# menyifang/MIMO

Measured on NVIDIA H100. Metric: frames/sec @ 512x512x24f, 20 DDIM steps, higher is better.
Workload: dtype fp16

## Files before the change

### include/mimo_b200.h

```cpp
#ifndef MIMO_B200_H_
#define MIMO_B200_H_

#include <stdint.h>

#ifdef __cplusplus
extern "C" {
#endif

#define MIMO_OK 0
#define MIMO_ERR_ARG (-1)
#define MIMO_ERR_CUDA (-2)
#define MIMO_ERR_DEVICE (-3)

#define MIMO_F16 0
#define MIMO_BF16 1

#define MIMO_ACT_NONE 0
#define MIMO_ACT_SILU 1
#define MIMO_ACT_GEGLU 2

const char* mimo_version(void);
const char* mimo_last_error(void);
int mimo_device_check(int dev);
int mimo_abi_sizeof(int which);
// ... 83 lines not shown
  void* out;
  int64_t ld_out;
  int32_t n, lq, heads, d;
  float scale;
  int32_t dtype;
} mimo_attn_params;
int mimo_attn_spatial(const mimo_attn_params* p, void* stream);

typedef struct {
  const void* q;
  int64_t ld_q;
  const void* k;
  const void* v;
  int64_t ld_kv;
  void* out;
  int64_t ld_out;
  int64_t chunk_stride_rows;
  int32_t batch, q_frames, kv_frames, frames_per_chunk;
  int32_t hw, heads, d;
  float scale;
  int32_t dtype;
} mimo_attn_temporal_params;
int mimo_attn_temporal(const mimo_attn_temporal_params* p, void* stream);

#define MIMO_MAX_PEERS 8
typedef struct {
  const void* peer_src[MIMO_MAX_PEERS];
  void* peer_ready[MIMO_MAX_PEERS];
  void* ctl;
  void* dst;
  const void* residual;
  int32_t mode, G, r;
  int32_t b, fl, hw, C;
  int32_t dtype;
  int32_t max_blocks;
  int32_t timeout_ms;
} mimo_exchange_params;
int mimo_exchange(const mimo_exchange_params* p, void* stream);
int mimo_peer_alloc(int64_t bytes, void** ptr, void* handle64);
int mimo_peer_open(const void* handle64, void** ptr);
int mimo_peer_close(void* ptr);
int mimo_peer_free(void* ptr);

int mimo_ncfhw_to_nhwc(const void* src, void* dst, int32_t b, int32_t c, int32_t f, int32_t h, int32_t w,
                       int32_t cpad, int32_t src_is_f32, int32_t dtype, void* stream);
int mimo_nhwc_to_ncfhw(const void* src, void* dst, int32_t b, int32_t c, int32_t f, int32_t h, int32_t w,
// ... 48 lines not shown
```

### mimo_b200/csrc/attn_temporal.cu

```cuda
#include <cuda_runtime.h>

#include "../../include/mimo_b200.h"
#include "host_util.h"
#include "ptx.cuh"

namespace mimo {

struct TemporalArgs {
  const void* q;
  const void* k;
  const void* v;
  void* out;
  long long ld_q, ld_kv, ld_out, chunk_stride_rows;
  int Fq, F, fpc, hw, heads, d;
  int dpad;
  int hg;
  int pitch;
  float scale_log2;
};

__device__ __forceinline__ void ldsm_x4(uint32_t (&r)[4], const void* p) {
  asm volatile("ldmatrix.sync.aligned.m8n8.x4.shared.b16 {%0, %1, %2, %3}, [%4];"
               : "=r"(r[0]), "=r"(r[1]), "=r"(r[2]), "=r"(r[3])
               : "r"(smem_u32(p)));
}
__device__ __forceinline__ void ldsm_x4_trans(uint32_t (&r)[4], const void* p) {
  asm volatile("ldmatrix.sync.aligned.m8n8.x4.trans.shared.b16 {%0, %1, %2, %3}, [%4];"
               : "=r"(r[0]), "=r"(r[1]), "=r"(r[2]), "=r"(r[3])
               : "r"(smem_u32(p)));
}
__device__ __forceinline__ void cp_async16(void* smem_dst, const void* gmem_src) {
  asm volatile("cp.async.cg.shared.global [%0], [%1], 16;" ::"r"(smem_u32(smem_dst)), "l"(gmem_src) : "memory");
}
template <bool kBf16>
__device__ __forceinline__ void mma16816(float (&c)[4], const uint32_t (&a)[4], uint32_t b0, uint32_t b1) {
  if constexpr (kBf16) {
    asm volatile("mma.sync.aligned.m16n8k16.row.col.f32.bf16.bf16.f32 {%0, %1, %2, %3}, {%4, %5, %6, %7}, {%8, %9}, "
                 "{%0, %1, %2, %3};"
                 : "+f"(c[0]), "+f"(c[1]), "+f"(c[2]), "+f"(c[3])
                 : "r"(a[0]), "r"(a[1]), "r"(a[2]), "r"(a[3]), "r"(b0), "r"(b1));
  } else {
    asm volatile("mma.sync.aligned.m16n8k16.row.col.f32.f16.f16.f32 {%0, %1, %2, %3}, {%4, %5, %6, %7}, {%8, %9}, "
                 "{%0, %1, %2, %3};"
                 : "+f"(c[0]), "+f"(c[1]), "+f"(c[2]), "+f"(c[3])
                 : "r"(a[0]), "r"(a[1]), "r"(a[2]), "r"(a[3]), "r"(b0), "r"(b1));
  }
}

template <bool kBf16, int D, int HG>
__global__ void __launch_bounds__(1024) attn_temporal_kernel(TemporalArgs a_in) {
  pdl_launch_dependents();
  pdl_wait();
  TemporalArgs a = a_in;
  if constexpr (D > 0) {
    a.d = D;
    a.dpad = (D + 15) / 16 * 16;
    a.hg = HG;
    a.pitch = HG * ((D + 15) / 16 * 16) + 8;
  }
  using C = Cvt<kBf16>;
  using T = typename C::T;
  extern __shared__ uint4 smem_qkv[];
  T* sq = reinterpret_cast<T*>(smem_qkv);
  T* sk = sq + 32 * a.pitch;
  T* sv = sk + 32 * a.pitch;
  const int groups = a.heads / a.hg;
  const int hg0 = (blockIdx.x % groups) * a.hg;
  const int bp = blockIdx.x / groups;
  const int b = bp / a.hw;
  const int p = bp % a.hw;
  const int d = a.d, dpad = a.dpad, pitch = a.pitch;
// ... 27 lines not shown
      }
    }
  }
  {
    const int warp = threadIdx.x >> 5, lane = threadIdx.x & 31, nwarps = blockDim.x >> 5;
    if (dpad > d) {
      const int padv = (dpad - d) / 8;
      for (int f = warp; f < 32; f += nwarps)
        for (int hh = lane; hh < a.hg; hh += 32)
          for (int pc = 0; pc < padv; ++pc) {
            *reinterpret_cast<uint4*>(sq + f * pitch + hh * dpad + d + pc * 8) = make_uint4(0, 0, 0, 0);
            *reinterpret_cast<uint4*>(sk + f * pitch + hh * dpad + d + pc * 8) = make_uint4(0, 0, 0, 0);
          }
    }
    for (int f = a.F + warp; f < 32; f += nwarps)
      for (int pc = lane; pc < pitch / 8; pc += 32) *reinterpret_cast<uint4*>(sv + f * pitch + pc * 8) = make_uint4(0, 0, 0, 0);
  }
  asm volatile("cp.async.wait_all;" ::: "memory");
  __syncthreads();

  const int hh = threadIdx.x >> 5;
  const int lane = threadIdx.x & 31;
  if (hh >= a.hg) return;
  const int g = lane >> 2, t = lane & 3;
  const int MT = (a.Fq + 15) >> 4;
  const int NT = (a.F + 7) >> 3;
  const bool ragged = (a.F & 7) != 0;
  const T* qh = sq + hh * dpad;
  const T* kh = sk + hh * dpad;
  const T* vh = sv + hh * dpad;

  float s[2][4][4];
#pragma unroll
  for (int mt = 0; mt < 2; ++mt)
#pragma unroll
    for (int nt = 0; nt < 4; ++nt)
#pragma unroll
      for (int e = 0; e < 4; ++e) s[mt][nt][e] = 0.f;
  for (int ks = 0; ks < dpad / 16; ++ks) {
    uint32_t af[2][4];
#pragma unroll
    for (int mt = 0; mt < 2; ++mt)
      if (mt < MT) ldsm_x4(af[mt], qh + (mt * 16 + (lane & 7) + ((lane >> 3) & 1) * 8) * pitch + ks * 16 + (lane >> 4) * 8);
#pragma unroll
    for (int np = 0; np < 2; ++np) {
      if (np * 2 < NT) {
        uint32_t bf[4];
        ldsm_x4(bf, kh + (np * 16 + (lane & 7) + (lane >> 4) * 8) * pitch + ks * 16 + ((lane >> 3) & 1) * 8);
#pragma unroll
        for (int mt = 0; mt < 2; ++mt) {
          if (mt < MT) {
            mma16816<kBf16>(s[mt][np * 2], af[mt], bf[0], bf[1]);
            if (np * 2 + 1 < NT) mma16816<kBf16>(s[mt][np * 2 + 1], af[mt], bf[2], bf[3]);
          }
        }
      }
    }
  }

  float inv_sum[2][2];
  uint32_t pf[2][2][4];
#pragma unroll
  for (int mt = 0; mt < 2; ++mt) {
#pragma unroll
    for (int half = 0; half < 2; ++half) {
      float m = -INFINITY;
#pragma unroll
      for (int nt = 0; nt < 4; ++nt) {
        if (nt < NT) {
#pragma unroll
          for (int e = 0; e < 2; ++e) {
            float& v = s[mt][nt][half * 2 + e];
            v *= a.scale_log2;
            if (ragged && nt == NT - 1 && nt * 8 + 2 * t + e >= a.F) v = -INFINITY;
            m = fmaxf(m, v);
          }
        }
      }
      m = fmaxf(m, __shfl_xor_sync(0xffffffffu, m, 1));
      m = fmaxf(m, __shfl_xor_sync(0xffffffffu, m, 2));
      float sum = 0.f;
#pragma unroll
      for (int nt = 0; nt < 4; ++nt) {
        if (nt < NT) {
#pragma unroll
          for (int e = 0; e < 2; ++e) {
            float& v = s[mt][nt][half * 2 + e];
            asm("ex2.approx.ftz.f32 %0, %1;" : "=f"(v) : "f"(v - m));
            sum += v;
          }
        }
      }
      sum += __shfl_xor_sync(0xffffffffu, sum, 1);
      sum += __shfl_xor_sync(0xffffffffu, sum, 2);
      inv_sum[mt][half] = 1.0f / sum;
    }
#pragma unroll
    for (int kk = 0; kk < 2; ++kk) {
      pf[mt][kk][0] = C::pack(s[mt][2 * kk][0], s[mt][2 * kk][1]);
      pf[mt][kk][1] = C::pack(s[mt][2 * kk][2], s[mt][2 * kk][3]);
      pf[mt][kk][2] = C::pack(s[mt][2 * kk + 1][0], s[mt][2 * kk + 1][1]);
      pf[mt][kk][3] = C::pack(s[mt][2 * kk + 1][2], s[mt][2 * kk + 1][3]);
    }
  }

  __syncwarp();
  T* oh = sq + hh * dpad;
  const int KK = (a.F + 15) >> 4;
  for (int nd = 0; nd < dv; ++nd) {
    uint32_t bv[4];
    ldsm_x4_trans(bv, vh + lane * pitch + nd * 8);
#pragma unroll
    for (int mt = 0; mt < 2; ++mt) {
      if (mt < MT) {
        float o[4] = {0.f, 0.f, 0.f, 0.f};
        mma16816<kBf16>(o, pf[mt][0], bv[0], bv[1]);
        if (KK > 1) mma16816<kBf16>(o, pf[mt][1], bv[2], bv[3]);
        *reinterpret_cast<uint32_t*>(oh + (mt * 16 + g) * pitch + nd * 8 + 2 * t) =
            C::pack(o[0] * inv_sum[mt][0], o[1] * inv_sum[mt][0]);
        *reinterpret_cast<uint32_t*>(oh + (mt * 16 + g + 8) * pitch + nd * 8 + 2 * t) =
            C::pack(o[2] * inv_sum[mt][1], o[3] * inv_sum[mt][1]);
      }
    }
  }
  __syncwarp();
  {
    const int lf = lane / dv, lpc = lane - lf * dv, fstep = 32 / dv;
    if (lf < fstep) {
      for (int f = lf; f < a.Fq; f += fstep) {
        const long long row = (static_cast<long long>(b) * a.Fq + f) * a.hw + p;
        *reinterpret_cast<uint4*>(static_cast<T*>(a.out) + row * a.ld_out + (hg0 + hh) * d + lpc * 8) =
            *reinterpret_cast<const uint4*>(oh + f * pitch + lpc * 8);
      }
    }
  }
}

}

using namespace mimo;

extern "C" int mimo_attn_temporal(const mimo_attn_temporal_params* p, void* stream) {
  if (!p || !p->q || !p->k || !p->v || !p->out) return set_error(MIMO_ERR_ARG, "mimo_attn_temporal: null pointer");
  const int fpc = p->frames_per_chunk > 0 ? p->frames_per_chunk : p->kv_frames;
  if (p->batch <= 0 || p->q_frames <= 0 || p->kv_frames <= 0 || p->kv_frames > 32 || p->q_frames > 32 || p->hw <= 0 ||
      p->heads <= 0 || p->heads > 32 || p->d <= 0 || (p->d % 8) || p->d > 256 || (p->ld_q % 8) || (p->ld_kv % 8) || (p->ld_out % 8) ||
      (p->kv_frames % fpc))
    return set_error(MIMO_ERR_ARG, "mimo_attn_temporal: need frames <= 32, heads <= 32, d % 8 == 0, kv_frames % chunk == 0");
// ... 55 lines not shown
```

### mimo_b200/csrc/capi.cu

```cuda
#include <cudaTypedefs.h>
#include <stdio.h>
#include <string.h>

#include "../../include/mimo_b200.h"
#include "host_util.h"

namespace mimo {

static thread_local char g_err[512] = "";

int set_error(int code, const char* msg) {
  snprintf(g_err, sizeof(g_err), "%s", msg);
  return code;
}
int set_cuda_error(const char* what, cudaError_t e) {
  snprintf(g_err, sizeof(g_err), "%s: %s (%s)", what, cudaGetErrorName(e), cudaGetErrorString(e));
  return MIMO_ERR_CUDA;
}

static int g_dev_state = 0;
static int g_num_sms = 132;

int ensure_device() {
  if (g_dev_state == 1) return MIMO_OK;
// ... 59 lines not shown
             (unsigned long long)(rank > 1 ? gdim[1] : 0), (unsigned long long)(rank > 2 ? gdim[2] : 0),
             (unsigned long long)(rank > 3 ? gdim[3] : 0), bx[0], rank > 1 ? bx[1] : 0, rank > 2 ? bx[2] : 0,
             rank > 3 ? bx[3] : 0, (unsigned long long)(rank > 1 ? gstr[0] : 0));
    return MIMO_ERR_CUDA;
  }
  return MIMO_OK;
}

}

extern "C" const char* mimo_version(void) { return "mimo_b200 0.2.0 (sm_90a)"; }
extern "C" const char* mimo_last_error(void) { return mimo::g_err; }

extern "C" int mimo_abi_sizeof(int which) {
  switch (which) {
    case 0: return static_cast<int>(sizeof(mimo_epilogue));
    case 1: return static_cast<int>(sizeof(mimo_gemm_params));
    case 2: return static_cast<int>(sizeof(mimo_conv3x3_params));
    case 3: return static_cast<int>(sizeof(mimo_groupnorm_params));
    case 4: return static_cast<int>(sizeof(mimo_attn_params));
    case 5: return static_cast<int>(sizeof(mimo_attn_temporal_params));
    case 6: return static_cast<int>(sizeof(mimo_exchange_params));
    case 7: return static_cast<int>(sizeof(mimo_cfg_multistep_params));
  }
  return -1;
}

extern "C" int mimo_device_check(int dev) {
  int count = 0;
  cudaError_t e = cudaGetDeviceCount(&count);
  if (e != cudaSuccess || count == 0) {
    mimo::set_error(MIMO_ERR_DEVICE, "no CUDA device visible; mimo_b200 has no CPU fallback");
    return MIMO_ERR_DEVICE;
  }
  if (dev < 0 || dev >= count) return mimo::set_error(MIMO_ERR_ARG, "mimo_device_check: bad device index");
  int major = 0, minor = 0;
  cudaDeviceGetAttribute(&major, cudaDevAttrComputeCapabilityMajor, dev);
  cudaDeviceGetAttribute(&minor, cudaDevAttrComputeCapabilityMinor, dev);
  if (major != 9 || minor != 0) return mimo::set_error(MIMO_ERR_DEVICE, "device is not sm_90 (H100)");
  return MIMO_OK;
}

extern "C" int mimo_peer_alloc(int64_t bytes, void** ptr, void* handle64) {
  if (!ptr || !handle64 || bytes <= 0) return mimo::set_error(MIMO_ERR_ARG, "mimo_peer_alloc: bad arguments");
  if (int rc = mimo::ensure_device()) return rc;
  void* p = nullptr;
// ... 40 lines not shown
```

### mimo_b200/engine.py

```python
from __future__ import annotations

import math
from dataclasses import dataclass
from typing import Dict, List, Optional, Sequence, Tuple

import torch

from . import lib as L
from . import ops

SD = Dict[str, torch.Tensor]


@dataclass
class UNetSpec:
    block_out_channels: Tuple[int, ...] = (320, 640, 1280, 1280)
    layers_per_block: int = 2
    heads: int = 8
    cross_attention_dim: int = 768
    norm_num_groups: int = 32
    norm_eps: float = 1e-5
    motion_groups: int = 32
    in_channels: int = 8
    out_channels: int = 4
# ... 237 lines not shown
        return ops.gemm(hcur, m["pout"][0], bias=m["pout"][1], residual=x)

    def _motion(self, p, x, b, f, hw):
        m = self.w[p]
        n = b * f
        xg = self.xchg
        G = xg.G if xg is not None else 1
        F_ = f * G
        if F_ > m["attn"][0]["pe"].shape[0]:
            raise L.MimoError(f"{F_} frames in a window exceed temporal_position_encoding_max_len="
                              f"{m['attn'][0]['pe'].shape[0]}")
        hcur = ops.groupnorm(x, *m["gn"], n, hw, groups=self.spec.motion_groups, eps=1e-6)
        C = m["pin"][0].shape[0]
        if G == 1:
            hw_l = hw
            hcur = ops.gemm(hcur, m["pin"][0], bias=m["pin"][1])
        else:
            if hw % G:
                raise L.MimoError(f"{hw} tokens per frame cannot be split over a frame group of {G} GPUs")
            hw_l = hw // G
            ops.gemm(hcur, m["pin"][0], out=xg.bufs["A"].view(n * hw, C, x.dtype), bias=m["pin"][1])
            hcur = xg.pull(0, "A", torch.empty((b * F_ * hw_l, C), dtype=x.dtype, device=x.device), b, f, hw, C)
        for a in m["attn"]:
            nh = ops.layernorm(hcur, *a["ln"], pe=a["pe"], rows_per_frame=hw_l, frames=F_)
            qkv = ops.gemm(nh, a["qkv"])
            att = ops.attn_temporal(qkv[:, :C], qkv[:, C:2 * C], qkv[:, 2 * C:], b, F_, hw_l, self.spec.heads)
            hcur = ops.gemm(att, a["o"][0], bias=a["o"][1], residual=hcur)
        hcur = self._ff(hcur, m["ffn"], m["geglu"], m["ffo"])
        if G == 1:
            return ops.gemm(hcur, m["pout"][0], bias=m["pout"][1], residual=x)
        ops.gemm(hcur, m["pout"][0], out=xg.bufs["B"].view(b * F_ * hw_l, C, x.dtype), bias=m["pout"][1])
        return xg.pull(1, "B", torch.empty_like(x), b, f, hw, C, residual=x)

    def _down(self, p, x, n, h, w):
        wp, b = self.w[p]
        col = ops.im2col3x3(x, n, h, w, stride=2)
        return ops.gemm(col, wp, bias=b)

    def _up(self, p, x, n, h, w, th, tw):
        if (th, tw) == (2 * h, 2 * w):
            wp, b = self.w[p]
            return ops.conv_up2x(x, wp, n, h, w, bias=b)
        wp, b = self.w[p + "_conv"]
        return ops.conv3x3(ops.upsample_nearest(x, n, h, w, th, tw), wp, n, th, tw, bias=b)

    def check_latent_size(self, h: int, w: int) -> None:
        m = 1 << (len(self.spec.block_out_channels) - 1)
        if h <= 0 or w <= 0 or h % m or w % m:
            raise L.MimoError(f"latent size {h} x {w} is not a multiple of {m} (pixels: {8 * m}): some up steps take the "
# ... 353 lines not shown
```

### mimo_b200/lib.py

```python
from __future__ import annotations

import ctypes as C
import os
from pathlib import Path

_PKG = Path(__file__).resolve().parent
LIB_PATH = _PKG / "libmimo_b200.so"

F16, BF16 = 0, 1
ACT_NONE, ACT_SILU, ACT_GEGLU = 0, 1, 2


class MimoError(RuntimeError):
    pass


class Epilogue(C.Structure):
    _fields_ = [
        ("bias", C.c_void_p),
        ("rowvec", C.c_void_p),
        ("rows_per_group", C.c_int64),
        ("ld_rowvec", C.c_int64),
        ("residual", C.c_void_p),
        ("ld_res", C.c_int64),
# ... 44 lines not shown

class AttnParams(C.Structure):
    _fields_ = [
        ("q", C.c_void_p), ("k", C.c_void_p), ("v", C.c_void_p), ("ld_qkv", C.c_int64),
        ("bank_k", C.c_void_p), ("bank_v", C.c_void_p), ("ld_bank", C.c_int64),
        ("lb", C.c_int32), ("nb", C.c_int32),
        ("bank_index", C.c_void_p),
        ("out", C.c_void_p), ("ld_out", C.c_int64),
        ("n", C.c_int32), ("lq", C.c_int32), ("heads", C.c_int32), ("d", C.c_int32),
        ("scale", C.c_float),
        ("dtype", C.c_int32),
    ]


class AttnTemporalParams(C.Structure):
    _fields_ = [
        ("q", C.c_void_p), ("ld_q", C.c_int64),
        ("k", C.c_void_p), ("v", C.c_void_p), ("ld_kv", C.c_int64),
        ("out", C.c_void_p), ("ld_out", C.c_int64),
        ("chunk_stride_rows", C.c_int64),
        ("batch", C.c_int32), ("q_frames", C.c_int32), ("kv_frames", C.c_int32), ("frames_per_chunk", C.c_int32),
        ("hw", C.c_int32), ("heads", C.c_int32), ("d", C.c_int32),
        ("scale", C.c_float),
        ("dtype", C.c_int32),
    ]


MAX_PEERS = 8


class ExchangeParams(C.Structure):
    _fields_ = [
        ("peer_src", C.c_void_p * MAX_PEERS), ("peer_ready", C.c_void_p * MAX_PEERS),
        ("ctl", C.c_void_p), ("dst", C.c_void_p), ("residual", C.c_void_p),
        ("mode", C.c_int32), ("G", C.c_int32), ("r", C.c_int32),
        ("b", C.c_int32), ("fl", C.c_int32), ("hw", C.c_int32), ("C", C.c_int32),
        ("dtype", C.c_int32), ("max_blocks", C.c_int32), ("timeout_ms", C.c_int32),
    ]


class CfgMultistepParams(C.Structure):
    _fields_ = [
        ("pred_uncond", C.c_void_p), ("pred_cond", C.c_void_p), ("counter", C.c_void_p), ("frame_stride", C.c_int64),
        ("latents", C.c_void_p), ("count", C.c_int64),
        ("hist_out", C.c_void_p), ("h1", C.c_void_p), ("h2", C.c_void_p), ("noise", C.c_void_p),
        ("guidance", C.c_float), ("a", C.c_float), ("b", C.c_float),
        ("c_x", C.c_float), ("c_m", C.c_float), ("c_1", C.c_float), ("c_2", C.c_float), ("c_n", C.c_float),
        ("dtype", C.c_int32),
    ]


_VP, _I32, _I64, _F = C.c_void_p, C.c_int32, C.c_int64, C.c_float
SYMBOLS = {
    "mimo_version": (C.c_char_p, []),
    "mimo_last_error": (C.c_char_p, []),
    "mimo_device_check": (C.c_int, [C.c_int]),
    "mimo_abi_sizeof": (C.c_int, [C.c_int]),
    "mimo_gemm": (C.c_int, [C.POINTER(GemmParams), _VP]),
    "mimo_gemm_geglu_granule": (C.c_int, [_I32]),
    "mimo_conv3x3": (C.c_int, [C.POINTER(Conv3x3Params), _VP]),
    "mimo_conv_up2x": (C.c_int, [C.POINTER(Conv3x3Params), _VP]),
    "mimo_im2col3x3": (C.c_int, [_VP, _VP, _I32, _I32, _I32, _I32, _I32, _I32, _I32, _I64, _I32, _VP]),
    "mimo_groupnorm": (C.c_int, [C.POINTER(GroupNormParams), _VP]),
    "mimo_groupnorm_workspace_bytes": (C.c_int64, [C.POINTER(GroupNormParams)]),
    "mimo_layernorm": (C.c_int, [_VP, _VP, _VP, _VP, _I64, _I32, _F, _VP, _I64, _I32, _I32, _I32, _VP]),
    "mimo_attn_spatial": (C.c_int, [C.POINTER(AttnParams), _VP]),
    "mimo_attn_temporal": (C.c_int, [C.POINTER(AttnTemporalParams), _VP]),
    "mimo_exchange": (C.c_int, [C.POINTER(ExchangeParams), _VP]),
    "mimo_peer_alloc": (C.c_int, [_I64, C.POINTER(C.c_void_p), C.c_char_p]),
    "mimo_peer_open": (C.c_int, [C.c_char_p, C.POINTER(C.c_void_p)]),
    "mimo_peer_close": (C.c_int, [_VP]),
    "mimo_peer_free": (C.c_int, [_VP]),
    "mimo_ncfhw_to_nhwc": (C.c_int, [_VP, _VP, _I32, _I32, _I32, _I32, _I32, _I32, _I32, _I32, _VP]),
    "mimo_nhwc_to_ncfhw": (C.c_int, [_VP, _VP, _I32, _I32, _I32, _I32, _I32, _I32, _I32, _I32, _VP]),
    "mimo_upsample2x": (C.c_int, [_VP, _VP, _I32, _I32, _I32, _I32, _I32, _VP]),
    "mimo_upsample_nearest": (C.c_int, [_VP, _VP, _I32, _I32, _I32, _I32, _I32, _I32, _I32, _VP]),
    "mimo_softmax_rows": (C.c_int, [_VP, _I64, _I32, _I64, _I32, _VP]),
    "mimo_add": (C.c_int, [_VP, _VP, _VP, _I64, _I32, _VP]),
    "mimo_silu": (C.c_int, [_VP, _VP, _I64, _I32, _VP]),
    "mimo_quick_gelu": (C.c_int, [_VP, _VP, _I64, _I32, _VP]),
    "mimo_composite_frame": (C.c_int, [_VP, _VP, _VP, _VP, _VP, _VP, C.c_double, _VP, _I64, _VP]),
    "mimo_cfg_ddim_step": (C.c_int, [_VP, _VP, _VP, _I64, _VP, _I64, _F, _F, _F, _F, _F, _I32, _VP]),
    "mimo_cfg_ddim_step_noise": (C.c_int, [_VP, _VP, _VP, _I64, _VP, _I64, _F, _F, _F, _F, _F, _VP, _F, _I32, _VP]),
    "mimo_interpolate_frames": (C.c_int, [_VP, _VP, _I32, _I64, _I32, _I32, _I32, _VP]),
    "mimo_cfg_multistep": (C.c_int, [C.POINTER(CfgMultistepParams), _VP]),
}
_DEBUG_SYMBOLS = {"mimo_debug_pdl": (C.c_int, [C.c_int]), "mimo_debug_splitk": (C.c_int, [C.c_int]),
                  "mimo_debug_force_bn": (C.c_int, [C.c_int])}

_lib = None


def load() -> C.CDLL:
    global _lib
    if _lib is not None:
        return _lib
    if not LIB_PATH.exists():
        raise MimoError(
            f"{LIB_PATH} is missing: run `python -m mimo_b200.build` (or __graft_entry__.build()). "
            "mimo_b200 has no CPU or PyTorch fallback."
        )
    lib = C.CDLL(os.fspath(LIB_PATH))
    for name, (res, args) in {**SYMBOLS, **_DEBUG_SYMBOLS}.items():
        fn = getattr(lib, name)
        fn.restype = res
        fn.argtypes = args
    for which, st in enumerate((Epilogue, GemmParams, Conv3x3Params, GroupNormParams, AttnParams, AttnTemporalParams,
                             ExchangeParams, CfgMultistepParams)):
        if lib.mimo_abi_sizeof(which) != C.sizeof(st):
            raise MimoError(f"ABI mismatch: {st.__name__} is {C.sizeof(st)} bytes in lib.py but "
                            f"{lib.mimo_abi_sizeof(which)} in {LIB_PATH.name}; rebuild the library")
    if os.environ.get("MIMO_B200_PDL") in ("0", "1"):
        lib.mimo_debug_pdl(int(os.environ["MIMO_B200_PDL"]))
    _lib = lib
    return lib


def check(rc: int, what: str = "") -> None:
    if rc != 0:
        msg = load().mimo_last_error().decode(errors="replace")
        raise MimoError(f"{what or 'mimo call'} failed (rc={rc}): {msg}")
```

### mimo_b200/ops.py

```python
from __future__ import annotations

import ctypes as C
from typing import List, Optional

import torch

from . import lib as L

_launches = 0
PROFILE: Optional[List[tuple]] = None


def launches() -> int:
    return _launches


def add_launches(k: int) -> None:
    global _launches
    _launches += k


class _Call:

    __slots__ = ("name", "k", "flops", "bytes", "e0")
# ... 231 lines not shown
                  frames_per_chunk: Optional[int] = None, chunk_stride_rows: int = 0) -> torch.Tensor:
    Cdim = q.shape[1]
    d = Cdim // heads
    fq = frames if q_frames is None else q_frames
    if out is None:
        out = torch.empty((batch * fq * hw, Cdim), dtype=q.dtype, device=q.device)
    p = L.AttnTemporalParams()
    p.q, p.ld_q = _ptr(q), q.stride(0)
    p.k, p.v, p.ld_kv = _ptr(k), _ptr(v), k.stride(0)
    assert k.stride(0) == v.stride(0)
    p.out, p.ld_out = _ptr(out), out.stride(0)
    p.chunk_stride_rows = int(chunk_stride_rows)
    p.batch, p.q_frames, p.kv_frames = batch, fq, frames
    p.frames_per_chunk = frames if frames_per_chunk is None else frames_per_chunk
    p.hw, p.heads, p.d = hw, heads, d
    p.scale = float(scale if scale is not None else d ** -0.5)
    p.dtype = _dt(q)
    rows = batch * fq * hw
    with _Call("attn_temporal", 1, 4.0 * rows * frames * Cdim, 2.0 * (2 * rows + 2 * batch * frames * hw) * Cdim):
        L.check(L.load().mimo_attn_temporal(C.byref(p), _stream()), "mimo_attn_temporal")
    return out


def exchange(xg, mode: int, name: str, dst: torch.Tensor, b: int, fl: int, hw: int, Cdim: int,
             residual: Optional[torch.Tensor] = None) -> torch.Tensor:
    assert dst.is_contiguous() and (residual is None or (residual.is_contiguous() and residual.shape == dst.shape))
    p = L.ExchangeParams()
    src, flags = xg.bufs[name], xg.flags
    for s in range(xg.G):
        p.peer_src[s] = src.peer_ptrs[s]
        p.peer_ready[s] = flags.peer_ptrs[s]
    p.ctl, p.dst, p.residual = _ptr(xg.ctl), _ptr(dst), _ptr(residual)
    p.mode, p.G, p.r = int(mode), xg.G, xg.r
    p.b, p.fl, p.hw, p.C = int(b), int(fl), int(hw), int(Cdim)
    p.dtype = _dt(dst)
    p.max_blocks, p.timeout_ms = int(xg.max_blocks), int(xg.timeout_ms)
    rows = b * fl * hw * (xg.G if mode == 2 else 1)
    need = b * fl * hw * Cdim * dst.element_size()
    if need > src.nbytes or dst.numel() != rows * Cdim:
        raise L.MimoError(f"exchange: source buffer '{name}' ({src.nbytes} B) or dst ({tuple(dst.shape)}) does not fit "
                          f"b={b} fl={fl} hw={hw} C={Cdim} mode={mode}")
    with _Call("exchange", 1, 0.0, 2.0 * dst.numel() * dst.element_size() + (dst.numel() * dst.element_size() if residual is not None else 0)):
        L.check(L.load().mimo_exchange(C.byref(p), _stream()), "mimo_exchange")
    return dst


# ... 190 lines not shown
```

Measured before the change: 8.150.

## Fuse temporal LayerNorm, QKV projection and attention into one warp-specialized kernel

Adds a single kernel that applies LayerNorm plus positional embedding to a tile of rows in shared memory, computes the per-head QKV projection with TMA-fed wgmma, and runs temporal attention per spatial position directly from shared memory. This removes the round trips through global memory for the normalized activations and the full QKV tensor, and saves two kernel launches per temporal attention block. The shared warp-level attention routine is factored into a header. The fused path covers only 320 channels with 8 heads and at most 32 frames, so other block widths fall back to the old three-kernel path. It also recomputes per-head loads across heads with a single block per SM, which may limit occupancy.

```diff
diff --git a/include/mimo_b200.h b/include/mimo_b200.h
--- a/include/mimo_b200.h
+++ b/include/mimo_b200.h
@@ -129,6 +129,20 @@
   int32_t dtype;
 } mimo_attn_temporal_params;
 int mimo_attn_temporal(const mimo_attn_temporal_params* p, void* stream);
+
+typedef struct {
+  const void* x;
+  const void* ln_gamma;
+  const void* ln_beta;
+  const void* pe;
+  const void* wqkv;
+  void* out;
+  int32_t batch, frames, hw, channels, heads;
+  float eps, scale;
+  int32_t dtype;
+} mimo_temporal_attn_qkv_params;
+int mimo_temporal_attn_qkv_supported(int32_t channels, int32_t heads, int32_t frames);
+int mimo_temporal_attn_qkv(const mimo_temporal_attn_qkv_params* p, void* stream);
 
 #define MIMO_MAX_PEERS 8
 typedef struct {
diff --git a/mimo_b200/csrc/attn_temporal.cu b/mimo_b200/csrc/attn_temporal.cu
--- a/mimo_b200/csrc/attn_temporal.cu
+++ b/mimo_b200/csrc/attn_temporal.cu
@@ -1,6 +1,7 @@
 #include <cuda_runtime.h>
 
 #include "../../include/mimo_b200.h"
+#include "attn_temporal_warp.cuh"
 #include "host_util.h"
 #include "ptx.cuh"
 
@@ -19,34 +20,9 @@
   float scale_log2;
 };
 
-__device__ __forceinline__ void ldsm_x4(uint32_t (&r)[4], const void* p) {
-  asm volatile("ldmatrix.sync.aligned.m8n8.x4.shared.b16 {%0, %1, %2, %3}, [%4];"
-               : "=r"(r[0]), "=r"(r[1]), "=r"(r[2]), "=r"(r[3])
-               : "r"(smem_u32(p)));
-}
-__device__ __forceinline__ void ldsm_x4_trans(uint32_t (&r)[4], const void* p) {
-  asm volatile("ldmatrix.sync.aligned.m8n8.x4.trans.shared.b16 {%0, %1, %2, %3}, [%4];"
-               : "=r"(r[0]), "=r"(r[1]), "=r"(r[2]), "=r"(r[3])
-               : "r"(smem_u32(p)));
-}
 __device__ __forceinline__ void cp_async16(void* smem_dst, const void* gmem_src) {
   asm volatile("cp.async.cg.shared.global [%0], [%1], 16;" ::"r"(smem_u32(smem_dst)), "l"(gmem_src) : "memory");
 }
-template <bool kBf16>
-__device__ __forceinline__ void mma16816(float (&c)[4], const uint32_t (&a)[4], uint32_t b0, uint32_t b1) {
-  if constexpr (kBf16) {
-    asm volatile("mma.sync.aligned.m16n8k16.row.col.f32.bf16.bf16.f32 {%0, %1, %2, %3}, {%4, %5, %6, %7}, {%8, %9}, "
-                 "{%0, %1, %2, %3};"
-                 : "+f"(c[0]), "+f"(c[1]), "+f"(c[2]), "+f"(c[3])
-                 : "r"(a[0]), "r"(a[1]), "r"(a[2]), "r"(a[3]), "r"(b0), "r"(b1));
-  } else {
-    asm volatile("mma.sync.aligned.m16n8k16.row.col.f32.f16.f16.f32 {%0, %1, %2, %3}, {%4, %5, %6, %7}, {%8, %9}, "
-                 "{%0, %1, %2, %3};"
-                 : "+f"(c[0]), "+f"(c[1]), "+f"(c[2]), "+f"(c[3])
-                 : "r"(a[0]), "r"(a[1]), "r"(a[2]), "r"(a[3]), "r"(b0), "r"(b1));
-  }
-}
-
 template <bool kBf16, int D, int HG>
 __global__ void __launch_bounds__(1024) attn_temporal_kernel(TemporalArgs a_in) {
   pdl_launch_dependents();
@@ -120,108 +96,8 @@
   const int hh = threadIdx.x >> 5;
   const int lane = threadIdx.x & 31;
   if (hh >= a.hg) return;
-  const int g = lane >> 2, t = lane & 3;
-  const int MT = (a.Fq + 15) >> 4;
-  const int NT = (a.F + 7) >> 3;
-  const bool ragged = (a.F & 7) != 0;
-  const T* qh = sq + hh * dpad;
-  const T* kh = sk + hh * dpad;
-  const T* vh = sv + hh * dpad;
-
-  float s[2][4][4];
-#pragma unroll
-  for (int mt = 0; mt < 2; ++mt)
-#pragma unroll
-    for (int nt = 0; nt < 4; ++nt)
-#pragma unroll
-      for (int e = 0; e < 4; ++e) s[mt][nt][e] = 0.f;
-  for (int ks = 0; ks < dpad / 16; ++ks) {
-    uint32_t af[2][4];
-#pragma unroll
-    for (int mt = 0; mt < 2; ++mt)
-      if (mt < MT) ldsm_x4(af[mt], qh + (mt * 16 + (lane & 7) + ((lane >> 3) & 1) * 8) * pitch + ks * 16 + (lane >> 4) * 8);
-#pragma unroll
-    for (int np = 0; np < 2; ++np) {
-      if (np * 2 < NT) {
-        uint32_t bf[4];
-        ldsm_x4(bf, kh + (np * 16 + (lane & 7) + (lane >> 4) * 8) * pitch + ks * 16 + ((lane >> 3) & 1) * 8);
-#pragma unroll
-        for (int mt = 0; mt < 2; ++mt) {
-          if (mt < MT) {
-            mma16816<kBf16>(s[mt][np * 2], af[mt], bf[0], bf[1]);
-            if (np * 2 + 1 < NT) mma16816<kBf16>(s[mt][np * 2 + 1], af[mt], bf[2], bf[3]);
-          }
-        }
-      }
-    }
-  }
-
-  float inv_sum[2][2];
-  uint32_t pf[2][2][4];
-#pragma unroll
-  for (int mt = 0; mt < 2; ++mt) {
-#pragma unroll
-    for (int half = 0; half < 2; ++half) {
-      float m = -INFINITY;
-#pragma unroll
-      for (int nt = 0; nt < 4; ++nt) {
-        if (nt < NT) {
-#pragma unroll
-          for (int e = 0; e < 2; ++e) {
-            float& v = s[mt][nt][half * 2 + e];
-            v *= a.scale_log2;
-            if (ragged && nt == NT - 1 && nt * 8 + 2 * t + e >= a.F) v = -INFINITY;
-            m = fmaxf(m, v);
-          }
-        }
-      }
-      m = fmaxf(m, __shfl_xor_sync(0xffffffffu, m, 1));
-      m = fmaxf(m, __shfl_xor_sync(0xffffffffu, m, 2));
-      float sum = 0.f;
-#pragma unroll
-      for (int nt = 0; nt < 4; ++nt) {
-        if (nt < NT) {
-#pragma unroll
-          for (int e = 0; e < 2; ++e) {
-            float& v = s[mt][nt][half * 2 + e];
-            asm("ex2.approx.ftz.f32 %0, %1;" : "=f"(v) : "f"(v - m));
-            sum += v;
-          }
-        }
-      }
-      sum += __shfl_xor_sync(0xffffffffu, sum, 1);
-      sum += __shfl_xor_sync(0xffffffffu, sum, 2);
-      inv_sum[mt][half] = 1.0f / sum;
-    }
-#pragma unroll
-    for (int kk = 0; kk < 2; ++kk) {
-      pf[mt][kk][0] = C::pack(s[mt][2 * kk][0], s[mt][2 * kk][1]);
-      pf[mt][kk][1] = C::pack(s[mt][2 * kk][2], s[mt][2 * kk][3]);
-      pf[mt][kk][2] = C::pack(s[mt][2 * kk + 1][0], s[mt][2 * kk + 1][1]);
-      pf[mt][kk][3] = C::pack(s[mt][2 * kk + 1][2], s[mt][2 * kk + 1][3]);
-    }
-  }
-
-  __syncwarp();
   T* oh = sq + hh * dpad;
-  const int KK = (a.F + 15) >> 4;
-  for (int nd = 0; nd < dv; ++nd) {
-    uint32_t bv[4];
-    ldsm_x4_trans(bv, vh + lane * pitch + nd * 8);
-#pragma unroll
-    for (int mt = 0; mt < 2; ++mt) {
-      if (mt < MT) {
-        float o[4] = {0.f, 0.f, 0.f, 0.f};
-        mma16816<kBf16>(o, pf[mt][0], bv[0], bv[1]);
-        if (KK > 1) mma16816<kBf16>(o, pf[mt][1], bv[2], bv[3]);
-        *reinterpret_cast<uint32_t*>(oh + (mt * 16 + g) * pitch + nd * 8 + 2 * t) =
-            C::pack(o[0] * inv_sum[mt][0], o[1] * inv_sum[mt][0]);
-        *reinterpret_cast<uint32_t*>(oh + (mt * 16 + g + 8) * pitch + nd * 8 + 2 * t) =
-            C::pack(o[2] * inv_sum[mt][1], o[3] * inv_sum[mt][1]);
-      }
-    }
-  }
-  __syncwarp();
+  temporal_attn_warp<kBf16>(oh, sk + hh * dpad, sv + hh * dpad, pitch, dpad, dv, a.Fq, a.F, a.scale_log2, 32);
   {
     const int lf = lane / dv, lpc = lane - lf * dv, fstep = 32 / dv;
     if (lf < fstep) {
diff --git a/mimo_b200/csrc/attn_temporal_fused.cu b/mimo_b200/csrc/attn_temporal_fused.cu
--- /dev/null
+++ b/mimo_b200/csrc/attn_temporal_fused.cu
@@ -0,0 +1,277 @@
+#include <cuda_runtime.h>
+
+#include <cudaTypedefs.h>
+
+#include "../../include/mimo_b200.h"
+#include "attn_temporal_warp.cuh"
+#include "host_util.h"
+#include "ptx.cuh"
+#include "wgmma.cuh"
+
+namespace mimo {
+
+namespace tf {
+constexpr int kC = 320, kHeads = 8, kD = 40, kDpad = 48;
+constexpr int kRows = 192;
+constexpr int kKB = kC / 64;
+constexpr int kN = 3 * kD;
+constexpr int kABytes = kRows * 128;
+constexpr int kStageBytes = kN * 128;
+constexpr int kStages = 3;
+constexpr int kPitch = 2 * kDpad + kD;
+constexpr int kSRows = kRows + 32;
+constexpr int kConsumers = 384;
+constexpr int kThreads = kConsumers + 32;
+constexpr int kSmem = kKB * kABytes + kStages * kStageBytes + kSRows * kPitch * 2 + 64;
+static_assert(kSmem <= 227 * 1024, "shared memory");
+}
+
+struct TfArgs {
+  const void* x;
+  const void* gamma;
+  const void* beta;
+  const void* pe;
+  void* out;
+  int F, hw, P, tiles;
+  float eps, scale_log2;
+};
+
+template <bool kBf16>
+__global__ void __launch_bounds__(tf::kThreads, 1)
+attn_temporal_fused_kernel(const __grid_constant__ CUtensorMap tmW, TfArgs a) {
+  using namespace tf;
+  using C = Cvt<kBf16>;
+  using T = typename C::T;
+  extern __shared__ __align__(1024) uint8_t smem[];
+  uint8_t* sA = smem;
+  uint8_t* sW = sA + kKB * kABytes;
+  T* sS = reinterpret_cast<T*>(sW + kStages * kStageBytes);
+  uint64_t* full_bar = reinterpret_cast<uint64_t*>(reinterpret_cast<uint8_t*>(sS) + kSRows * kPitch * 2);
+  uint64_t* empty_bar = full_bar + kStages;
+
+  pdl_launch_dependents();
+  const int warp = __shfl_sync(0xffffffffu, threadIdx.x >> 5, 0);
+  const int lane = threadIdx.x & 31;
+  if (warp == 12 && lane == 0) {
+    tma_prefetch_desc(&tmW);
+    for (int s = 0; s < kStages; ++s) {
+      mbar_init(&full_bar[s], 1);
+      mbar_init(&empty_bar[s], kConsumers / 32);
+    }
+    fence_mbar_init();
+  }
+  __syncthreads();
+  pdl_wait();
+
+  const int bb = blockIdx.x / a.tiles;
+  const int p0 = (blockIdx.x % a.tiles) * a.P;
+
+  if (warp == 12) {
+    uint32_t stage = 0, phase = 0;
+    for (int h = 0; h < kHeads; ++h) {
+      for (int kb = 0; kb < kKB; ++kb) {
+        mbar_wait(&empty_bar[stage], phase ^ 1u);
+        if (elect_one()) {
+          uint8_t* dst = sW + stage * kStageBytes;
+          mbar_expect_tx(&full_bar[stage], kStageBytes);
+#pragma unroll
+          for (int part = 0; part < 3; ++part)
+            tma_load_2d(dst + part * kD * 128, &tmW, &full_bar[stage], kb * 64, part * kC + h * kD);
+        }
+        __syncwarp();
+        if (++stage == kStages) {
+          stage = 0;
+          phase ^= 1u;
+        }
+      }
+    }
+    return;
+  }
+
+  const int ct = threadIdx.x;
+  for (int i = ct; i < kSRows * 2; i += kConsumers) {
+    const int r = i >> 1;
+    *reinterpret_cast<uint4*>(sS + r * kPitch + (i & 1) * kDpad + kD) = make_uint4(0, 0, 0, 0);
+  }
+  for (int i = ct; i < 32 * (kPitch / 8); i += kConsumers)
+    *reinterpret_cast<uint4*>(sS + (kRows + i / (kPitch / 8)) * kPitch + (i % (kPitch / 8)) * 8) = make_uint4(0, 0, 0, 0);
+
+  {
+    constexpr int L = 8;
+    constexpr int Cdim = kC;
+    const int sub = lane % L;
+    const int rsel = ct / L;
+#pragma unroll 1
+    for (int it = 0; it < kRows / 48; ++it) {
+      const int r = it * 48 + rsel;
+      const int pl = r / a.F, f = r - pl * a.F;
+      const bool ok = pl < a.P && p0 + pl < a.hw;
+      const long long row = (static_cast<long long>(bb) * a.F + f) * a.hw + p0 + pl;
+      const T* xr = static_cast<const T*>(a.x) + row * Cdim;
+      uint4 u[5];
+      float sum = 0.f;
+#pragma unroll
+      for (int j = 0; j < 5; ++j) {
+        u[j] = ok ? *reinterpret_cast<const uint4*>(xr + (sub + j * L) * 8) : make_uint4(0, 0, 0, 0);
+        const uint32_t w[4] = {u[j].x, u[j].y, u[j].z, u[j].w};
+#pragma unroll
+        for (int k = 0; k < 4; ++k) {
+          const float2 t = C::unpack(w[k]);
+          sum += t.x + t.y;
+        }
+      }
+#pragma unroll
+      for (int o = L / 2; o > 0; o >>= 1) sum += __shfl_xor_sync(0xffffffffu, sum, o);
+      const float mean = sum * (1.0f / Cdim);
+      float sq = 0.f;
+#pragma unroll
+      for (int j = 0; j < 5; ++j) {
+        const uint32_t w[4] = {u[j].x, u[j].y, u[j].z, u[j].w};
+#pragma unroll
+        for (int k = 0; k < 4; ++k) {
+          const float2 t = C::unpack(w[k]);
+          const float d0 = t.x - mean, d1 = t.y - mean;
+          sq += d0 * d0 + d1 * d1;
+        }
+      }
+#pragma unroll
+      for (int o = L / 2; o > 0; o >>= 1) sq += __shfl_xor_sync(0xffffffffu, sq, o);
+      const float rstd = rsqrtf(sq * (1.0f / Cdim) + a.eps);
+      const T* per = static_cast<const T*>(a.pe) + f * Cdim;
+#pragma unroll
+      for (int j = 0; j < 5; ++j) {
+        const int v = sub + j * L;
+        const uint32_t w[4] = {u[j].x, u[j].y, u[j].z, u[j].w};
+        const uint4 up = __ldg(reinterpret_cast<const uint4*>(per + v * 8));
+        const uint4 ug = __ldg(reinterpret_cast<const uint4*>(static_cast<const T*>(a.gamma) + v * 8));
+        const uint4 ub = __ldg(reinterpret_cast<const uint4*>(static_cast<const T*>(a.beta) + v * 8));
+        const uint32_t wp[4] = {up.x, up.y, up.z, up.w};
+        const uint32_t wg[4] = {ug.x, ug.y, ug.z, ug.w};
+        const uint32_t wb[4] = {ub.x, ub.y, ub.z, ub.w};
+        uint32_t o[4];
+#pragma unroll
+        for (int k = 0; k < 4; ++k) {
+          const float2 t = C::unpack(w[k]);
+          const float2 g2 = C::unpack(wg[k]);
+          const float2 b2 = C::unpack(wb[k]);
+          float y0 = (t.x - mean) * rstd * g2.x + b2.x;
+          float y1 = (t.y - mean) * rstd * g2.y + b2.y;
+          const float2 p2 = C::unpack(wp[k]);
+          y0 = C::to_f(C::from_f(y0)) + p2.x;
+          y1 = C::to_f(C::from_f(y1)) + p2.y;
+          o[k] = C::pack(y0, y1);
+        }
+        const uint4 val = ok ? make_uint4(o[0], o[1], o[2], o[3]) : make_uint4(0, 0, 0, 0);
+        *reinterpret_cast<uint4*>(sA + j * kABytes + r * 128 + ((sub ^ (r & 7)) << 4)) = val;
+      }
+    }
+  }
+  fence_proxy_async_smem();
+  bar_sync(1, kConsumers);
+
+  const int wg = warp >> 2;
+  const int rbase = wg * 64 + (warp & 3) * 16 + (lane >> 2);
+  const int q2 = (lane & 3) * 2;
+  float acc[kN / 2];
+  uint32_t stage = 0, phase = 0;
+#pragma unroll 1
+  for (int h = 0; h < kHeads; ++h) {
+    uint32_t prev_stage = 0;
+#pragma unroll 1
+    for (int kb = 0; kb < kKB; ++kb) {
+      mbar_wait(&full_bar[stage], phase);
+      const uint64_t da = make_smem_desc_sw128(smem_u32(sA + kb * kABytes + wg * (64 * 128)), 16, 1024);
+      const uint64_t db = make_smem_desc_sw128(smem_u32(sW + stage * kStageBytes), 16, 1024);
+      wgmma_fence();
+#pragma unroll
+      for (int k = 0; k < 4; ++k) Wgmma<kN, kBf16>::ss(acc, da + 2 * k, db + 2 * k, (kb | k) != 0 ? 1u : 0u);
+      wgmma_commit();
+      if (kb > 0) {
+        wgmma_wait<1>();
+        if (lane == 0) mbar_arrive(&empty_bar[prev_stage]);
+      }
+      prev_stage = stage;
+      if (++stage == kStages) {
+        stage = 0;
+        phase ^= 1u;
+      }
+    }
+    wgmma_wait<0>();
+    reg_fence(acc);
+    if (lane == 0) mbar_arrive(&empty_bar[prev_stage]);
+
+    bar_sync(1, kConsumers);
+#pragma unroll
+    for (int j = 0; j < kN / 8; ++j) {
+      const int part = j / (kD / 8);
+      const int col = part * kDpad + (8 * j - part * kD) + q2;
+#pragma unroll
+      for (int hh = 0; hh < 2; ++hh)
+        *reinterpret_cast<uint32_t*>(sS + (rbase + 8 * hh) * kPitch + col) = C::pack(acc[4 * j + 2 * hh], acc[4 * j + 2 * hh + 1]);
+    }
+    bar_sync(1, kConsumers);
+
+    for (int pl = warp; pl < a.P; pl += kConsumers / 32) {
+      if (p0 + pl >= a.hw) break;
+      T* qh = sS + pl * a.F * kPitch;
+      temporal_attn_warp<kBf16>(qh, qh + kDpad, qh + 2 * kDpad, kPitch, kDpad, kD / 8, a.F, a.F, a.scale_log2, a.F);
+      const int lf = lane / 5, lpc = lane - lf * 5;
+      if (lf < 6) {
+        for (int f = lf; f < a.F; f += 6) {
+          const long long row = (static_cast<long long>(bb) * a.F + f) * a.hw + p0 + pl;
+          *reinterpret_cast<uint4*>(static_cast<T*>(a.out) + row * kC + h * kD + lpc * 8) =
+              *reinterpret_cast<const uint4*>(qh + f * kPitch + lpc * 8);
+        }
+      }
+    }
+  }
+}
+
+}
+
+using namespace mimo;
+
+extern "C" int mimo_temporal_attn_qkv_supported(int32_t channels, int32_t heads, int32_t frames) {
+  return channels == tf::kC && heads == tf::kHeads && frames >= 1 && frames <= 32;
+}
+
+extern "C" int mimo_temporal_attn_qkv(const mimo_temporal_attn_qkv_params* p, void* stream) {
+  if (!p || !p->x || !p->ln_gamma || !p->ln_beta || !p->pe || !p->wqkv || !p->out)
+    return set_error(MIMO_ERR_ARG, "mimo_temporal_attn_qkv: null pointer");
+  if (!mimo_temporal_attn_qkv_supported(p->channels, p->heads, p->frames) || p->batch <= 0 || p->hw <= 0)
+    return set_error(MIMO_ERR_ARG, "mimo_temporal_attn_qkv: needs channels 320, 8 heads, 1 <= frames <= 32");
+  if (int rc = ensure_device()) return rc;
+  TfArgs a;
+  a.x = p->x;
+  a.gamma = p->ln_gamma;
+  a.beta = p->ln_beta;
+  a.pe = p->pe;
+  a.out = p->out;
+  a.F = p->frames;
+  a.hw = p->hw;
+  a.P = tf::kRows / p->frames;
+  a.tiles = static_cast<int>(div_up(p->hw, a.P));
+  a.eps = p->eps;
+  a.scale_log2 = p->scale * 1.4426950408889634f;
+  const long long nblk = static_cast<long long>(p->batch) * a.tiles;
+  if (nblk > 0x7fffffffLL) return set_error(MIMO_ERR_ARG, "mimo_temporal_attn_qkv: grid too large");
+  CUtensorMap tmW;
+  const uint64_t wdim[2] = {static_cast<uint64_t>(tf::kC), static_cast<uint64_t>(3 * tf::kC)};
+  const uint64_t wstr[1] = {static_cast<uint64_t>(tf::kC) * 2};
+  const uint32_t wbox[2] = {64, static_cast<uint32_t>(tf::kD)};
+  if (int rc = encode_tmap(&tmW, p->dtype, 2, p->wqkv, wdim, wstr, wbox)) return rc;
+  cudaStream_t st = static_cast<cudaStream_t>(stream);
+  const bool bf = p->dtype == MIMO_BF16;
+  static bool attr_done[2] = {};
+  void (*kern)(const CUtensorMap, TfArgs) = bf ? attn_temporal_fused_kernel<true> : attn_temporal_fused_kernel<false>;
+  cudaError_t e = cudaSuccess;
+  if (!attr_done[bf]) {
+    e = cudaFuncSetAttribute(kern, cudaFuncAttributeMaxDynamicSharedMemorySize, tf::kSmem);
+    if (e != cudaSuccess) return set_cuda_error("temporal_attn_qkv attr", e);
+    attr_done[bf] = true;
+  }
+  e = launch_k(kern, dim3(static_cast<unsigned>(nblk)), dim3(tf::kThreads), tf::kSmem, st, tmW, a);
+  if (e == cudaSuccess) e = cudaGetLastError();
+  if (e != cudaSuccess) return set_cuda_error("temporal_attn_qkv launch", e);
+  return MIMO_OK;
+}
diff --git a/mimo_b200/csrc/attn_temporal_warp.cuh b/mimo_b200/csrc/attn_temporal_warp.cuh
--- /dev/null
+++ b/mimo_b200/csrc/attn_temporal_warp.cuh
@@ -0,0 +1,139 @@
+#pragma once
+#include "ptx.cuh"
+
+namespace mimo {
+
+__device__ __forceinline__ void ldsm_x4(uint32_t (&r)[4], const void* p) {
+  asm volatile("ldmatrix.sync.aligned.m8n8.x4.shared.b16 {%0, %1, %2, %3}, [%4];"
+               : "=r"(r[0]), "=r"(r[1]), "=r"(r[2]), "=r"(r[3])
+               : "r"(smem_u32(p)));
+}
+__device__ __forceinline__ void ldsm_x4_trans(uint32_t (&r)[4], const void* p) {
+  asm volatile("ldmatrix.sync.aligned.m8n8.x4.trans.shared.b16 {%0, %1, %2, %3}, [%4];"
+               : "=r"(r[0]), "=r"(r[1]), "=r"(r[2]), "=r"(r[3])
+               : "r"(smem_u32(p)));
+}
+template <bool kBf16>
+__device__ __forceinline__ void mma16816(float (&c)[4], const uint32_t (&a)[4], uint32_t b0, uint32_t b1) {
+  if constexpr (kBf16) {
+    asm volatile("mma.sync.aligned.m16n8k16.row.col.f32.bf16.bf16.f32 {%0, %1, %2, %3}, {%4, %5, %6, %7}, {%8, %9}, "
+                 "{%0, %1, %2, %3};"
+                 : "+f"(c[0]), "+f"(c[1]), "+f"(c[2]), "+f"(c[3])
+                 : "r"(a[0]), "r"(a[1]), "r"(a[2]), "r"(a[3]), "r"(b0), "r"(b1));
+  } else {
+    asm volatile("mma.sync.aligned.m16n8k16.row.col.f32.f16.f16.f32 {%0, %1, %2, %3}, {%4, %5, %6, %7}, {%8, %9}, "
+                 "{%0, %1, %2, %3};"
+                 : "+f"(c[0]), "+f"(c[1]), "+f"(c[2]), "+f"(c[3])
+                 : "r"(a[0]), "r"(a[1]), "r"(a[2]), "r"(a[3]), "r"(b0), "r"(b1));
+  }
+}
+
+template <bool kBf16>
+__device__ __forceinline__ void temporal_attn_warp(typename Cvt<kBf16>::T* qh, const typename Cvt<kBf16>::T* kh,
+                                                   const typename Cvt<kBf16>::T* vh, int pitch, int dpad, int dv, int Fq,
+                                                   int F, float scale_log2, int o_rows) {
+  using C = Cvt<kBf16>;
+  const int lane = threadIdx.x & 31;
+  const int g = lane >> 2, t = lane & 3;
+  const int MT = (Fq + 15) >> 4;
+  const int NT = (F + 7) >> 3;
+  const bool ragged = (F & 7) != 0;
+
+  float s[2][4][4];
+#pragma unroll
+  for (int mt = 0; mt < 2; ++mt)
+#pragma unroll
+    for (int nt = 0; nt < 4; ++nt)
+#pragma unroll
+      for (int e = 0; e < 4; ++e) s[mt][nt][e] = 0.f;
+  for (int ks = 0; ks < dpad / 16; ++ks) {
+    uint32_t af[2][4];
+#pragma unroll
+    for (int mt = 0; mt < 2; ++mt)
+      if (mt < MT) ldsm_x4(af[mt], qh + (mt * 16 + (lane & 7) + ((lane >> 3) & 1) * 8) * pitch + ks * 16 + (lane >> 4) * 8);
+#pragma unroll
+    for (int np = 0; np < 2; ++np) {
+      if (np * 2 < NT) {
+        uint32_t bf[4];
+        ldsm_x4(bf, kh + (np * 16 + (lane & 7) + (lane >> 4) * 8) * pitch + ks * 16 + ((lane >> 3) & 1) * 8);
+#pragma unroll
+        for (int mt = 0; mt < 2; ++mt) {
+          if (mt < MT) {
+            mma16816<kBf16>(s[mt][np * 2], af[mt], bf[0], bf[1]);
+            if (np * 2 + 1 < NT) mma16816<kBf16>(s[mt][np * 2 + 1], af[mt], bf[2], bf[3]);
+          }
+        }
+      }
+    }
+  }
+
+  float inv_sum[2][2];
+  uint32_t pf[2][2][4];
+#pragma unroll
+  for (int mt = 0; mt < 2; ++mt) {
+#pragma unroll
+    for (int half = 0; half < 2; ++half) {
+      float m = -INFINITY;
+#pragma unroll
+      for (int nt = 0; nt < 4; ++nt) {
+        if (nt < NT) {
+#pragma unroll
+          for (int e = 0; e < 2; ++e) {
+            float& v = s[mt][nt][half * 2 + e];
+            v *= scale_log2;
+            if (ragged && nt == NT - 1 && nt * 8 + 2 * t + e >= F) v = -INFINITY;
+            m = fmaxf(m, v);
+          }
+        }
+      }
+      m = fmaxf(m, __shfl_xor_sync(0xffffffffu, m, 1));
+      m = fmaxf(m, __shfl_xor_sync(0xffffffffu, m, 2));
+      float sum = 0.f;
+#pragma unroll
+      for (int nt = 0; nt < 4; ++nt) {
+        if (nt < NT) {
+#pragma unroll
+          for (int e = 0; e < 2; ++e) {
+            float& v = s[mt][nt][half * 2 + e];
+            asm("ex2.approx.ftz.f32 %0, %1;" : "=f"(v) : "f"(v - m));
+            sum += v;
+          }
+        }
+      }
+      sum += __shfl_xor_sync(0xffffffffu, sum, 1);
+      sum += __shfl_xor_sync(0xffffffffu, sum, 2);
+      inv_sum[mt][half] = 1.0f / sum;
+    }
+#pragma unroll
+    for (int kk = 0; kk < 2; ++kk) {
+      pf[mt][kk][0] = C::pack(s[mt][2 * kk][0], s[mt][2 * kk][1]);
+      pf[mt][kk][1] = C::pack(s[mt][2 * kk][2], s[mt][2 * kk][3]);
+      pf[mt][kk][2] = C::pack(s[mt][2 * kk + 1][0], s[mt][2 * kk + 1][1]);
+      pf[mt][kk][3] = C::pack(s[mt][2 * kk + 1][2], s[mt][2 * kk + 1][3]);
+    }
+  }
+
+  __syncwarp();
+  const int KK = (F + 15) >> 4;
+  for (int nd = 0; nd < dv; ++nd) {
+    uint32_t bv[4];
+    ldsm_x4_trans(bv, vh + lane * pitch + nd * 8);
+#pragma unroll
+    for (int mt = 0; mt < 2; ++mt) {
+      if (mt < MT) {
+        float o[4] = {0.f, 0.f, 0.f, 0.f};
+        mma16816<kBf16>(o, pf[mt][0], bv[0], bv[1]);
+        if (KK > 1) mma16816<kBf16>(o, pf[mt][1], bv[2], bv[3]);
+        if (mt * 16 + g < o_rows)
+          *reinterpret_cast<uint32_t*>(qh + (mt * 16 + g) * pitch + nd * 8 + 2 * t) =
+              C::pack(o[0] * inv_sum[mt][0], o[1] * inv_sum[mt][0]);
+        if (mt * 16 + g + 8 < o_rows)
+          *reinterpret_cast<uint32_t*>(qh + (mt * 16 + g + 8) * pitch + nd * 8 + 2 * t) =
+              C::pack(o[2] * inv_sum[mt][1], o[3] * inv_sum[mt][1]);
+      }
+    }
+  }
+  __syncwarp();
+}
+
+}
diff --git a/mimo_b200/csrc/capi.cu b/mimo_b200/csrc/capi.cu
--- a/mimo_b200/csrc/capi.cu
+++ b/mimo_b200/csrc/capi.cu
@@ -105,6 +105,7 @@
     case 5: return static_cast<int>(sizeof(mimo_attn_temporal_params));
     case 6: return static_cast<int>(sizeof(mimo_exchange_params));
     case 7: return static_cast<int>(sizeof(mimo_cfg_multistep_params));
+    case 8: return static_cast<int>(sizeof(mimo_temporal_attn_qkv_params));
   }
   return -1;
 }
diff --git a/mimo_b200/engine.py b/mimo_b200/engine.py
--- a/mimo_b200/engine.py
+++ b/mimo_b200/engine.py
@@ -283,9 +283,7 @@
             ops.gemm(hcur, m["pin"][0], out=xg.bufs["A"].view(n * hw, C, x.dtype), bias=m["pin"][1])
             hcur = xg.pull(0, "A", torch.empty((b * F_ * hw_l, C), dtype=x.dtype, device=x.device), b, f, hw, C)
         for a in m["attn"]:
-            nh = ops.layernorm(hcur, *a["ln"], pe=a["pe"], rows_per_frame=hw_l, frames=F_)
-            qkv = ops.gemm(nh, a["qkv"])
-            att = ops.attn_temporal(qkv[:, :C], qkv[:, C:2 * C], qkv[:, 2 * C:], b, F_, hw_l, self.spec.heads)
+            att = ops.temporal_attn_qkv(hcur, *a["ln"], a["pe"], a["qkv"], b, F_, hw_l, self.spec.heads)
             hcur = ops.gemm(att, a["o"][0], bias=a["o"][1], residual=hcur)
         hcur = self._ff(hcur, m["ffn"], m["geglu"], m["ffo"])
         if G == 1:
diff --git a/mimo_b200/lib.py b/mimo_b200/lib.py
--- a/mimo_b200/lib.py
+++ b/mimo_b200/lib.py
@@ -90,6 +90,16 @@
         ("batch", C.c_int32), ("q_frames", C.c_int32), ("kv_frames", C.c_int32), ("frames_per_chunk", C.c_int32),
         ("hw", C.c_int32), ("heads", C.c_int32), ("d", C.c_int32),
         ("scale", C.c_float),
+        ("dtype", C.c_int32),
+    ]
+
+
+class TemporalAttnQkvParams(C.Structure):
+    _fields_ = [
+        ("x", C.c_void_p), ("ln_gamma", C.c_void_p), ("ln_beta", C.c_void_p), ("pe", C.c_void_p),
+        ("wqkv", C.c_void_p), ("out", C.c_void_p),
+        ("batch", C.c_int32), ("frames", C.c_int32), ("hw", C.c_int32), ("channels", C.c_int32), ("heads", C.c_int32),
+        ("eps", C.c_float), ("scale", C.c_float),
         ("dtype", C.c_int32),
     ]
 
@@ -134,6 +144,8 @@
     "mimo_layernorm": (C.c_int, [_VP, _VP, _VP, _VP, _I64, _I32, _F, _VP, _I64, _I32, _I32, _I32, _VP]),
     "mimo_attn_spatial": (C.c_int, [C.POINTER(AttnParams), _VP]),
     "mimo_attn_temporal": (C.c_int, [C.POINTER(AttnTemporalParams), _VP]),
+    "mimo_temporal_attn_qkv_supported": (C.c_int, [_I32, _I32, _I32]),
+    "mimo_temporal_attn_qkv": (C.c_int, [C.POINTER(TemporalAttnQkvParams), _VP]),
     "mimo_exchange": (C.c_int, [C.POINTER(ExchangeParams), _VP]),
     "mimo_peer_alloc": (C.c_int, [_I64, C.POINTER(C.c_void_p), C.c_char_p]),
     "mimo_peer_open": (C.c_int, [C.c_char_p, C.POINTER(C.c_void_p)]),
@@ -174,7 +186,7 @@
         fn.restype = res
         fn.argtypes = args
     for which, st in enumerate((Epilogue, GemmParams, Conv3x3Params, GroupNormParams, AttnParams, AttnTemporalParams,
-                             ExchangeParams, CfgMultistepParams)):
+                             ExchangeParams, CfgMultistepParams, TemporalAttnQkvParams)):
         if lib.mimo_abi_sizeof(which) != C.sizeof(st):
             raise MimoError(f"ABI mismatch: {st.__name__} is {C.sizeof(st)} bytes in lib.py but "
                             f"{lib.mimo_abi_sizeof(which)} in {LIB_PATH.name}; rebuild the library")
diff --git a/mimo_b200/ops.py b/mimo_b200/ops.py
--- a/mimo_b200/ops.py
+++ b/mimo_b200/ops.py
@@ -277,6 +277,28 @@
     return out
 
 
+def temporal_attn_qkv(x: torch.Tensor, gamma: torch.Tensor, beta: torch.Tensor, pe: torch.Tensor, wqkv: torch.Tensor,
+                      batch: int, frames: int, hw: int, heads: int, *, eps=1e-5) -> torch.Tensor:
+    assert x.is_contiguous() and x.dim() == 2 and wqkv.is_contiguous() and pe.is_contiguous()
+    Cdim = x.shape[1]
+    if not L.load().mimo_temporal_attn_qkv_supported(Cdim, heads, frames):
+        nh = layernorm(x, gamma, beta, eps=eps, pe=pe, rows_per_frame=hw, frames=frames)
+        qkv = gemm(nh, wqkv)
+        return attn_temporal(qkv[:, :Cdim], qkv[:, Cdim:2 * Cdim], qkv[:, 2 * Cdim:], batch, frames, hw, heads)
+    assert wqkv.shape == (3 * Cdim, Cdim) and x.shape[0] == batch * frames * hw and pe.shape[0] >= frames
+    out = torch.empty_like(x)
+    p = L.TemporalAttnQkvParams()
+    p.x, p.ln_gamma, p.ln_beta, p.pe, p.wqkv, p.out = (_ptr(t) for t in (x, gamma, beta, pe, wqkv, out))
+    p.batch, p.frames, p.hw, p.channels, p.heads = batch, frames, hw, Cdim, heads
+    p.eps, p.scale = float(eps), float((Cdim // heads) ** -0.5)
+    p.dtype = _dt(x)
+    rows = x.shape[0]
+    with _Call("temporal_attn_qkv", 1, 2.0 * rows * 3 * Cdim * Cdim + 4.0 * rows * frames * Cdim,
+               2.0 * (2 * rows * Cdim + 3 * Cdim * Cdim)):
+        L.check(L.load().mimo_temporal_attn_qkv(C.byref(p), _stream()), "mimo_temporal_attn_qkv")
+    return out
+
+
 def exchange(xg, mode: int, name: str, dst: torch.Tensor, b: int, fl: int, hw: int, Cdim: int,
              residual: Optional[torch.Tensor] = None) -> torch.Tensor:
     assert dst.is_contiguous() and (residual is None or (residual.is_contiguous() and residual.shape == dst.shape))
```

New measurement: 8.324 (median of 6 runs). +2.1%, better.
